# peterzjx/DeepHall

Hardware: AMD Instinct MI355X
Metric: local-energies/sec + MCMC walker-steps/sec, N=6 2Q=15, 1/2/4/8 GPUs (higher is better)
Workload: dtype f32; 1 GPU; VMC iteration (mcmc_step 10 MH moves + local energy + stats all-reduce), nspins=[6, 0] flux=15, Psiformer 4x64 heads, 2 layers, 1 det; walkers_per_gpu=4096, global_batch=4096, parallelism=walker-dp1, walker_groups_per_gpu=1, gemm_arithmetic=x6all

## Files before the change

deephall_amd/_lib.py:

```python

from __future__ import annotations

import ctypes as C
import os
from pathlib import Path

LIB_PATH = Path(__file__).resolve().parent / "_lib" / "libdeephall_amd.so"

DH_NSTATS = 16
STAT_NAMES = [
    "energy_re",
    "energy_im",
    "clipped_re",
    "clipped_im",
    "ere2",
    "kinetic_re",
    "kinetic_im",
    "potential",
    "angular_momentum_z",
    "angular_momentum_z_square",
    "angular_momentum_square",
    "pmove",
    "nvalid",
    "clipped_lz2",
# ... 18 lines not shown
    "dh_loss_diff",
    "dh_init_walkers",
    "dh_potential",
    "dh_histograms",
    "dh_monopole_orbitals",
    "dh_mh_init",
    "dh_mh_propose",
    "dh_mh_accept",
    "dh_kinetic_from_derivatives",
    "dh_debug_trunk",
    "dh_debug_gemm",
    "dh_debug_gemm_ln",
    "dh_debug_gemm_x6_ln",
    "dh_debug_chain_x6",
    "dh_debug_gemm_lnch",
    "dh_debug_set_lnch_form",
    "dh_debug_x6_plane_rows",
    "dh_debug_split_planes",
    "dh_debug_gemm_x6",
    "dh_debug_gemm_x6_choice",
    "dh_debug_route",
    "dh_debug_set_det_in_chain",
    "dh_debug_det_in_chain",
    "dh_ref_layout",
    "dh_set_params_ref",
    "dh_vjp_workspace_bytes",
    "dh_logpsi_vjp",
    "dh_grad_cotangent",
    "dh_adam_update",
    "dh_profile_enable",
    "dh_profile_read",
    "dh_debug_f_offset",
    "dh_debug_env_leaf",
    "dh_kfac_layout",
    "dh_kfac_workspace_bytes",
    "dh_kfac_vjp",
    "dh_kfac_step",
    "dh_ntk_workspace_bytes",
    "dh_ntk_tile_walkers",
    "dh_ntk",
    "dh_ntk_part",
    "dh_ntk_mirror",
    "dh_ntk_owner",
    "dh_minsr_matrix_workspace_bytes",
    "dh_minsr_matrix",
    "dh_ntk_jvp_workspace_bytes",
# ... 95 lines not shown
    lib.dh_debug_gemm_ln.restype = i32
    lib.dh_debug_gemm_x6_ln.argtypes = [i32, i32, vp, i32, vp, i32, vp, vp, vp, i32, i32, vp]
    lib.dh_debug_gemm_x6_ln.restype = i32
    lib.dh_debug_chain_x6.argtypes = [vp, vp, i32, vp, vp, vp, i32, vp, vp, vp, i32, vp, i32, vp, i32, vp, i32, vp]
    lib.dh_debug_chain_x6.restype = i32
    lib.dh_debug_gemm_lnch.argtypes = [i32, i32, vp, vp, i32, vp, vp, vp, vp, i32, vp]
    lib.dh_debug_gemm_lnch.restype = i32
    lib.dh_debug_set_lnch_form.argtypes = [i32]
    lib.dh_debug_set_lnch_form.restype = i32
    lib.dh_debug_x6_plane_rows.argtypes = [i32]
    lib.dh_debug_x6_plane_rows.restype = i32
    lib.dh_debug_split_planes.argtypes = [vp, i32, i32, i32, vp, vp]
    lib.dh_debug_split_planes.restype = i32
    lib.dh_debug_gemm_x6.argtypes = [i32, vp, i32, vp, i32, vp, vp, i32, vp, i32, i32, i32, i32, i32, vp]
    lib.dh_debug_gemm_x6.restype = i32
    lib.dh_debug_gemm_x6_choice.argtypes = [i32, i32]
    lib.dh_debug_gemm_x6_choice.restype = i32
    lib.dh_debug_route.argtypes = [vp, i32, i32, C.POINTER(i32), i32]
    lib.dh_debug_route.restype = i32
    lib.dh_debug_set_det_in_chain.argtypes = [i32]
    lib.dh_debug_set_det_in_chain.restype = i32
    lib.dh_debug_det_in_chain.argtypes = [vp, i32, i32]
    lib.dh_debug_det_in_chain.restype = i32
    lib.dh_ref_layout.argtypes = [vp, C.POINTER(sz), i32]
    lib.dh_ref_layout.restype = i32
    lib.dh_set_params_ref.argtypes = [vp, vp, sz, vp]
    lib.dh_set_params_ref.restype = i32
    lib.dh_vjp_workspace_bytes.argtypes = [vp, i32]
    lib.dh_vjp_workspace_bytes.restype = sz
    lib.dh_logpsi_vjp.argtypes = [vp, vp, i32, vp, vp, vp, vp, sz, vp]
    lib.dh_logpsi_vjp.restype = i32
    lib.dh_kfac_layout.argtypes = [vp, C.POINTER(sz), i32]
    lib.dh_kfac_layout.restype = i32
    lib.dh_kfac_workspace_bytes.argtypes = [vp, i32]
    lib.dh_kfac_workspace_bytes.restype = sz
    lib.dh_kfac_vjp.argtypes = [vp, vp, i32, vp, vp, vp, vp, vp, sz, vp]
    lib.dh_kfac_vjp.restype = i32
    lib.dh_kfac_step.argtypes = [vp, vp, vp, f32, f32, vp, vp, f32, f32, f32, vp, vp, vp, sz, vp]
    lib.dh_kfac_step.restype = i32
    lib.dh_ntk_workspace_bytes.argtypes = [vp, i32]
    lib.dh_ntk_workspace_bytes.restype = sz
    lib.dh_ntk_tile_walkers.argtypes = [vp]
    lib.dh_ntk_tile_walkers.restype = i32
    lib.dh_ntk.argtypes = [vp, vp, i32, vp, vp, vp, vp, sz, vp]
    lib.dh_ntk.restype = i32
    lib.dh_ntk_part.argtypes = [vp, vp, i32, vp, vp, vp, vp, sz, i32, i32, vp]
# ... 42 lines not shown
```

deephall_amd/csrc/api.cpp:

```cpp
#include <cmath>
#include <cstring>

#include "api_internal.h"

using namespace dh;

thread_local std::string dh::g_err;

namespace {

struct Work {
  float *h, *qkv, *o, *t, *F, *geo, *x2, *logpsi, *lp;
  int32_t* nacc;
  size_t total_bytes;
  TrunkRoute route;
};

size_t env_first_floats(const Dims& d, int nw) {
  const size_t ne = (size_t)nw * d.N, r6 = (size_t)round_up((int)(6 * ne), 256), r1 = (size_t)round_up((int)ne, 256);
  return align64(r6 * 256) + align64(r6 * d.ld_orb) + align64(r1 * env_first_k(d)) + align64(r1 * 256 * 2 * d.N);
}

Work carve(const Dims& d, int gemm_mode, int nw, int C, void* base) {
  const int rows = nw * d.N * C;
// ... 579 lines not shown
  return DH_OK;
}

size_t dh_workspace_bytes(const dh_handle* h, int batch, int op) {
  if (!h || batch < 1) return 0;
  return carve(h->d, h->gemm_mode, batch, op == 1 ? h->d.C : 1, nullptr).total_bytes;
}

}

namespace {

struct Trunk {
  dh_handle* h;
  const Dims& d;
  const Params& P;
  const Work& w;
  hipStream_t s;
  const int nw, C, rows;
  const TrunkRoute r;
  const bool keep_h;
  const ChainDet* det = nullptr;
  const bool keep_F = false;
  const int D = d.D, KO = ofeat_k(d);
  const int ch = C > 1 ? PK_CH : 0;
  const double R = rows, DD = D, f4 = 4.0;

  void gemm(const float* X, int ldx, const float* W, const float* Wt, const uint16_t* Wp, int ldw, const float* bias,
            const float* Res, int ldr, float* Y, int ldy, int ncols, int K) const {
    PROF(PK_GEMM + ch, 2.0 * R * ncols * K, f4 * (R * K + (double)K * ncols + R * ncols * (Res ? 2 : 1)));
    dense_gemm(r.family, X, ldx, W, Wt, Wp, ldw, bias, Res, ldr, Y, ldy, rows, ncols, K, C, s);
  }
  X6Feat h0_feat(int l) const { return (r.h0_epilogue && l == 0) ? X6Feat{P.W0, w.geo, d.N, d.n_up} : X6Feat{}; }

  void layer_chain(int l, bool attn) const {
    const LayerParams& lp = P.layer[l];
    const bool last = l + 1 == d.L;
    const int n3 = last ? d.orb_cols : 3 * D;
    PROF(PK_GEMM, 2.0 * R * DD * (2.0 * DD + n3), f4 * (2.0 * R * DD + R * n3 + 2.0 * DD * DD + DD * n3));
    X6Feat feat = h0_feat(l);
    if (attn) {
      feat.W0qkv = P.W0qkv;
      feat.bqkv = lp.bqkv;
      feat.Mqk = P.Mqk;
      feat.L1V = P.L1VP;
      feat.L1B = P.L1BP;
    }
    launch_chain_x6(w.o, attn ? P.UP : lp.WolP, x6_plane_rows(D), lp.bol, lp.ln1, lp.WmP, x6_plane_rows(D), lp.bm,
                    lp.ln2, last ? P.WorbP : P.layer[l + 1].WqkvP, x6_plane_rows(n3),
                    last ? P.borb : P.layer[l + 1].bqkv, n3, last ? w.F : w.qkv, last ? d.ld_orb : 3 * D, w.h, rows,
                    feat, s, !last || keep_h,
                    last ? det : nullptr, !(last && det) || keep_F);
  }
  void layer_ln_epilogue(int l) const {
    const LayerParams& lp = P.layer[l];
    const bool x6 = r.family == GEMM_X6;
    {
      PROF(PK_GEMM, 2.0 * R * DD * DD, f4 * (3.0 * R * DD + DD * DD));
      if (x6)
        launch_gemm_x6_ln(w.o, D, lp.WolP, x6_plane_rows(D), lp.bol, lp.ln1, w.h, rows, D, 0, 0, s, h0_feat(l));
      else
        launch_gemm_ln(w.o, D, lp.WolT, D, lp.bol, lp.ln1, w.h, rows, D, 0, 0, s);
    }
    PROF(PK_GEMM, 2.0 * R * DD * DD, f4 * (2.0 * R * DD + DD * DD));
    if (x6)
      launch_gemm_x6_ln(w.h, D, lp.WmP, x6_plane_rows(D), lp.bm, lp.ln2, w.h, rows, D, 1, 0, s);
    else
      launch_gemm_ln(w.h, D, lp.WmT, D, lp.bm, lp.ln2, w.h, rows, D, 1, 0, s);
  }
  void layer_lnch(int l) const {
    const LayerParams& lp = P.layer[l];
    {
      const bool of = r.ofeat && l == 0;
      const double KK = of ? KO : DD;
      PROF(PK_GEMM + PK_CH, 2.0 * R * DD * KK, f4 * (R * KK + 2.0 * R * DD + DD * KK));
// ... 22 lines not shown
    else
      gemm(w.o, D, lp.Wol, lp.WolT, lp.WolP, D, lp.bol, lf ? nullptr : w.h, D, w.t, D, D, D);
    {
      PROF(PK_LN + ch, 0.0, f4 * R * 2.0 * DD);
      launch_layernorm(d, w.t, nullptr, lp.ln1, w.geo, w.h, nw, C, 0, s, lf ? P.W0 : nullptr);
    }
    gemm(w.h, D, lp.Wm, lp.WmT, lp.WmP, D, lp.bm, nullptr, 0, w.o, D, D, D);
    PROF(PK_LN + ch, 0.0, f4 * R * 3.0 * DD);
    launch_layernorm(d, nullptr, w.o, lp.ln2, w.geo, w.h, nw, C, 1, s);
  }

  int run(const float* x, bool geo_ready) const {
    if (!(geo_ready && r.input_skip)) {
      const bool wq = r.input_qkv;
      PROF(PK_INPUT + ch, 8.0 * R * DD * (wq ? 4 : 1), f4 * R * DD * (wq ? 4 : 1));
      launch_input(d, x, P.W0, wq ? P.W0qkv : nullptr, wq ? P.layer[0].bqkv : nullptr, r.input_h ? w.h : nullptr,
                   wq ? w.qkv : nullptr, w.geo, nw, C, s);
    }
    for (int l = 0; l < d.L; ++l) {
      const LayerParams& lp = P.layer[l];
      const int form = l == 0 ? r.form0 : r.form1;
      if (l > 0 && r.qkv_gemm)
        gemm(w.h, D, lp.Wqkv, lp.WqkvT, lp.WqkvP, 3 * D, lp.bqkv, nullptr, 0, w.qkv, 3 * D, 3 * D, D);
      if (form != LF_CHAIN_ATTN) {
        const bool f = r.attn_feat && l == 0;
        PROF(PK_ATTN + ch, 0.0, f4 * R * (f ? 1.0 : 4.0) * DD);
        launch_attention(d, w.qkv, w.geo, w.o, nw, C, s, f ? P.W0qkv : nullptr, f ? lp.bqkv : nullptr,
                         f ? P.Mqk : nullptr);
      }
      switch (form) {
        case LF_CHAIN:
        case LF_CHAIN_ATTN: layer_chain(l, form == LF_CHAIN_ATTN); break;
        case LF_LN_EPILOGUE: layer_ln_epilogue(l); break;
        case LF_LNCH_WHOLE: layer_lnch_whole(); break;
        case LF_LNCH_PAIR: layer_lnch(l); break;
        case LF_L1CH: layer_l1ch(); break;
        default: layer_separate(l); break;
      }
    }
    if (r.orbital == ORB_GEMM)
      gemm(w.h, D, P.Worb, P.WorbT, P.WorbP, d.ld_orb, P.borb, nullptr, 0, w.F, d.ld_orb, d.orb_cols, D);
    return check_launch();
  }
};

int run_trunk(dh_handle* h, const float* x, int nw, int C, const Work& w, hipStream_t s, bool geo_ready = false,
              bool keep_h = false, const ChainDet* det = nullptr, bool keep_F = false) {
  return Trunk{h, h->d, h->p, w, s, nw, C, nw * h->d.N * C, w.route, keep_h, det, keep_F}.run(x, geo_ready);
}

ChainDet chain_det(const dh_handle* h, const float* x, int nw, float* logpsi, const McmcEpi& epi) {
  const Dims& d = h->d;
  ChainDet c;
  c.x = x;
  c.jastrow = h->p.jastrow;
  c.norm = h->norm;
  c.logpsi = logpsi;
  c.N = d.N;
  c.n_up = d.n_up;
  c.M = d.M;
  c.K = d.K;
  c.nw = nw;
  c.per = det_value_per(d);
  c.ldf = det_chain_ldf(d);
  c.epi = epi;
  return c;
}

int launch_trial(dh_handle* h, const float* x, float* logpsi, float* e_l, float* obs, int nw, hipStream_t s) {
  if (!h->expo && !h->expo_host.empty()) {
    HIP_TRY(hipMalloc(&h->expo, h->expo_host.size() * sizeof(int)));
    HIP_TRY(hipMemcpy(h->expo, h->expo_host.data(), h->expo_host.size() * sizeof(int), hipMemcpyHostToDevice));
  }
  PROF(e_l ? PK_DET_ENERGY : PK_DET_VALUE, 0.0, e_l ? 48.0 * nw : 8.0 * nw * h->d.N);
  if (h->state == dh_handle::PFAFFIAN)
    launch_pfaffian(h->d, x, h->cfg.cf_flux, logpsi, e_l, obs, nw, s);
  else if (h->state == dh_handle::JAIN)
    launch_cf(h->d, x, h->expo, h->cf_dense, logpsi, e_l, obs, nw, s);
  else
    launch_laughlin(h->d, x, h->expo, logpsi, e_l, obs, nw, s);
  return check_launch();
}

int value_pass(dh_handle* h, const float* x, int nw, const Work& w, float* logpsi, hipStream_t s,
               bool geo_ready = false, const McmcEpi& epi = McmcEpi{}) {
  if (h->analytic()) return launch_trial(h, x, logpsi, nullptr, nullptr, nw, s);
  if (w.route.det_in_chain && !h->prof.on) {
    const ChainDet det = chain_det(h, x, nw, logpsi, epi);
    return run_trunk(h, x, nw, 1, w, s, geo_ready, false, &det);
  }
  if (int rc = run_trunk(h, x, nw, 1, w, s, geo_ready)) return rc;
  {
    PROF(PK_DET_VALUE, 0.0, 4.0 * nw * h->d.N * h->d.ld_orb);
    launch_det_value(h->d, w.F, x, h->p.jastrow, h->norm, logpsi, nw, s, epi);
  }
  return check_launch();
}

}

extern "C" {

int dh_logpsi(dh_handle* h, const float* x, int B, float* logpsi, void* ws, size_t ws_bytes, void* stream) {
  const size_t need = h ? dh_workspace_bytes(h, B, 0) : 0;
  if (int rc = check_common(h, x, B, ws, ws_bytes, need)) return rc;
  if (!logpsi) return fail(DH_EINVAL, "null output");
  hipStream_t s = (hipStream_t)stream;
  Work w = carve(h->d, h->gemm_mode, B, 1, ws);
  return value_pass(h, x, B, w, logpsi, s);
}

int dh_mcmc_step(dh_handle* h, float* x, float* lp, int32_t* n_accept, int B, int steps, float width, uint64_t seed,
                 uint64_t counter, int64_t walker_offset, const float* noise, void* ws, size_t ws_bytes,
                 void* stream) {
// ... 124 lines not shown

int dh_fidelity_partial(const float* logpsi, const float* logphi, int B, double* part, void* stream) {
  if (!logpsi || !logphi || !part) return fail(DH_EINVAL, "dh_fidelity_partial: null argument");
  if (B < 1) return fail(DH_EINVAL, "dh_fidelity_partial needs B >= 1");
  launch_fidelity_partial(logpsi, logphi, B, part, (hipStream_t)stream);
  return check_launch();
}

int dh_fidelity_residual(const float* logpsi, const float* logphi, int B, const double* total, float* resid,
                         void* stream) {
  if (!logpsi || !logphi || !total || !resid) return fail(DH_EINVAL, "dh_fidelity_residual: null argument");
  if (B < 1) return fail(DH_EINVAL, "dh_fidelity_residual needs B >= 1");
  launch_fidelity_residual(logpsi, logphi, B, total, resid, (hipStream_t)stream);
  return check_launch();
}

int dh_debug_trunk(dh_handle* h, const float* x, int B, int op, void* ws, size_t ws_bytes, void* stream) {
  const size_t need = h ? dh_workspace_bytes(h, B, op) : 0;
  if (int rc = check_common(h, x, B, ws, ws_bytes, need)) return rc;
  Work w = carve(h->d, h->gemm_mode, B, op == 1 ? h->d.C : 1, ws);
  if (!w.F)
    return fail(DH_EINVAL, "dh_debug_trunk: this config's local energy goes envelope first and maps no orbital "
                           "features F over the channel rows");
  if (op != 1 && w.route.det_in_chain) {
    const ChainDet det = chain_det(h, x, B, w.logpsi, McmcEpi{});
    return run_trunk(h, x, B, 1, w, (hipStream_t)stream, false, true, &det, true);
  }
  return run_trunk(h, x, B, op == 1 ? h->d.C : 1, w, (hipStream_t)stream, false, true);
}

int dh_debug_env_leaf(const float* thph, int n, int M, int sq, float* out, void* stream) {
  if (!thph || !out || n < 1 || M < 1) return fail(DH_EINVAL, "bad env_leaf probe args");
  launch_env_leaf_probe(thph, n, M, sq, out, (hipStream_t)stream);
  return check_launch();
}

size_t dh_debug_f_offset(const dh_handle* h, int B, int op) {
  if (!h || B < 1) return (size_t)-1;
  Work w = carve(h->d, h->gemm_mode, B, op == 1 ? h->d.C : 1, reinterpret_cast<void*>(size_t(64)));
  if (!w.F) return (size_t)-1;
  return (size_t)(w.F - reinterpret_cast<float*>(size_t(64)));
}

int dh_debug_gemm(int variant, const float* X, int ldx, const float* W, int ldw, const float* bias, const float* R,
                  int ldr, float* Y, int ldy, int rows, int ncols, int K, int C, void* stream) {
  bool known = true;
  if (variant >= 100) {
    if (K % 32 != 0) return fail(DH_EINVAL, "NT GEMM needs K % 32 == 0");
    known = launch_gemm_nt_variant(variant - 100, X, ldx, W, ldw, bias, R, ldr, Y, ldy, rows, ncols, K, C,
                                   (hipStream_t)stream);
  } else {
// ... 49 lines not shown
    return fail(DH_EINVAL, "bad chain_x6 args");
  launch_chain_x6(X1, Wp1, ldp1, b1, ln1, Wp2, ldp2, b2, ln2, Wp3, ldp3, b3, n3, Y3, ldy3, h, rows, X6Feat{},
                  (hipStream_t)stream);
  return check_launch();
}

int dh_debug_gemm_lnch(int N, int mode, const float* X, const uint16_t* Wp, int ldp, const float* bias,
                       const float* ln, const float* geo, float* h, int ne, void* stream) {
  if (!gemm_lnch_supported(N, 256) || (mode != 0 && mode != 1) || (mode == 0 && !X) || !Wp || !ln || !geo || !h ||
      ne < 1 || ldp < x6_plane_rows(256) || ne % N)
    return fail(DH_EINVAL, "bad gemm_lnch args");
  launch_gemm_lnch(N, mode == 0 ? X : h, Wp, ldp, bias, ln, geo, h, ne, mode, (hipStream_t)stream);
  return check_launch();
}

int dh_debug_set_lnch_form(int form) { return set_lnch_form(form); }

int dh_debug_set_det_in_chain(int on) { return set_det_in_chain(on); }

int dh_debug_det_in_chain(const dh_handle* h, int B, int op) {
  if (!h || h->analytic() || B < 1) return fail(DH_EINVAL, "bad route query");
  const int C = op == 1 ? h->d.C : 1;
  return trunk_route(h->d, h->gemm_mode, C, B * h->d.N * C).det_in_chain;
}

int dh_debug_gemm_ln(int mode, int bm, const float* X, int ldx, const float* Wt, int ldw, const float* bias,
                     const float* ln, float* h, int rows, int K, void* stream) {
  if (!gemm_ln_supported(256, K) || rows < 1 || (mode != 0 && mode != 1)) return fail(DH_EINVAL, "bad gemm_ln args");
  launch_gemm_ln(X, ldx, Wt, ldw, bias, ln, h, rows, K, mode, bm, (hipStream_t)stream);
  return check_launch();
}

int dh_profile_enable(dh_handle* h, int on) {
  if (!h) return fail(DH_EINVAL, "null handle");
  h->prof.on = on != 0;
  h->prof.used = 0;
  return DH_OK;
}

int dh_profile_read(dh_handle* h, double* out, int reset) {
  if (!h || !out) return fail(DH_EINVAL, "null argument");
  for (int i = 0; i < 4 * PK_TOTAL; ++i) out[i] = 0.0;
  for (size_t i = 0; i < h->prof.used; ++i) {
    ProfRec& r = h->prof.recs[i];
    HIP_TRY(hipEventSynchronize(r.b));
    float ms = 0.f;
// ... 73 lines not shown
```

deephall_amd/csrc/attn_val.h:

```cpp
#pragma once
#include "device_common.h"

namespace dh {

struct FeatW {
  float4 wq, wk, wv;
  float bq, bk, bv;
  __device__ void load(const float* W0qkv, const float* bqkv, int D, int col) {
    const int ld = 3 * D;
    wq = make_float4(W0qkv[col], W0qkv[ld + col], W0qkv[2 * ld + col], W0qkv[3 * ld + col]);
    wk = make_float4(W0qkv[D + col], W0qkv[ld + D + col], W0qkv[2 * ld + D + col], W0qkv[3 * ld + D + col]);
    wv = make_float4(W0qkv[2 * D + col], W0qkv[ld + 2 * D + col], W0qkv[2 * ld + 2 * D + col],
                     W0qkv[3 * ld + 2 * D + col]);
    bq = bqkv[col];
    bk = bqkv[D + col];
    bv = bqkv[2 * D + col];
  }
  __device__ __forceinline__ static float dot(float4 f, float4 w) {
    return fmaf(f.x, w.x, fmaf(f.y, w.y, fmaf(f.z, w.z, f.w * w.w)));
  }
};

template <int N>
__device__ __forceinline__ void feat_qkv(const FeatW& fw, const float* __restrict__ geo, int b, int n_up,
                                         float (&pq)[N], float (&pk)[N], float (&pv)[N]) {
#pragma unroll
  for (int i = 0; i < N; ++i) {
    const float4 g = *reinterpret_cast<const float4*>(geo + 4 * (size_t)(b * N + i));
    const float4 f = make_float4(g.y, g.x * g.w, g.x * g.z, (i < n_up) ? 1.f : -1.f);
    pq[i] = FeatW::dot(f, fw.wq) + fw.bq;
    pk[i] = FeatW::dot(f, fw.wk) + fw.bk;
    pv[i] = FeatW::dot(f, fw.wv) + fw.bv;
  }
}

template <int N>
__host__ __device__ constexpr int attn_val_floats() { return 2 * N * 68 + N * N; }

template <int N, int NT>
__device__ __forceinline__ void attn_val_core(const float (&pq)[NT][N], const float (&pk)[NT][N],
                                              const float (&pv)[NT][N], float* st, int lane, float (&out)[NT][N]) {
  constexpr int ld = 68, nn = N * N, PER = attn_val_floats<N>();
  __builtin_amdgcn_wave_barrier();
#pragma unroll
  for (int t = 0; t < NT; ++t)
#pragma unroll
    for (int i = 0; i < N; ++i) {
      st[t * PER + i * ld + lane] = pq[t][i];
      st[t * PER + N * ld + i * ld + lane] = pk[t][i];
    }
  __builtin_amdgcn_wave_barrier();
  for (int p = lane; p < NT * 4 * nn; p += 64) {
    const int t = p / (4 * nn), pp = p - t * (4 * nn);
    const int pair = pp >> 2, qt = pp & 3, i = pair / N, j = pair - (pair / N) * N;
    const float* x = st + t * PER + i * ld + 16 * qt;
    const float* y = st + t * PER + N * ld + j * ld + 16 * qt;
    float sdot = 0.f;
#pragma unroll
    for (int m = 0; m < 4; ++m) {
      const float4 a = *reinterpret_cast<const float4*>(x + 4 * m);
      const float4 c = *reinterpret_cast<const float4*>(y + 4 * m);
      sdot = fmaf(a.x, c.x, fmaf(a.y, c.y, fmaf(a.z, c.z, fmaf(a.w, c.w, sdot))));
    }
    sdot += __shfl_xor(sdot, 1, 64);
    sdot += __shfl_xor(sdot, 2, 64);
    if (qt == 0) st[t * PER + 2 * N * ld + pair] = sdot * 0.125f;
  }
  __builtin_amdgcn_wave_barrier();
  if (lane < NT * N) {
    const int t = lane / N, r = lane - t * N;
    float* A = st + t * PER + 2 * N * ld + r * N;
    float m = -INFINITY;
#pragma unroll
    for (int j = 0; j < N; ++j) m = fmaxf(m, A[j]);
// ... 153 lines not shown
```

deephall_amd/csrc/dh_internal.h:

```cpp
#pragma once
#include <algorithm>
#include <hip/hip_runtime.h>
#include <stdint.h>
#include <stddef.h>

#include "../../include/deephall_amd.h"

namespace dh {

struct Dims {
  int N, n_up, n_dn;
  int T;
  int C;
  int M;
  float Q, r;
  int H, dh, D, L, K;
  int NB;
  int orb_cols;
  int ld_orb;
  int interaction;
  float lambda;
  int sparse;
};
constexpr int kSparseFeatures = 8;
// ... 37 lines not shown
  LF_SEPARATE = 0,
  LF_LN_EPILOGUE,
  LF_CHAIN,
  LF_CHAIN_ATTN,
  LF_LNCH_PAIR,
  LF_LNCH_WHOLE,
  LF_L1CH,
};
enum OrbitalMap : int { ORB_NONE = 0, ORB_GEMM = 1, ORB_IN_CHAIN = 2 };
enum DetStage : int { DET_VALUE = 0, DET_DIRECT = 1, DET_PRECONTRACT = 2, DET_ENV_FIRST = 3 };
struct TrunkRoute {
  int family;
  int input_h;
  int input_qkv;
  int input_skip;
  int form0, form1;
  int attn_feat;
  int h0_epilogue;
  int ofeat;
  int qkv_gemm;
  int orbital;
  int det;
  int det_in_chain;
};
constexpr int kTrunkRouteFields = 12;
static_assert(sizeof(TrunkRoute) == (kTrunkRouteFields + 1) * sizeof(int) &&
                  offsetof(TrunkRoute, det_in_chain) == kTrunkRouteFields * sizeof(int),
              "dh_debug_route copies the first kTrunkRouteFields fields as ints");
int gemm_family(const Dims& d, bool want_x6);
TrunkRoute trunk_route(const Dims& d, int gemm_mode, int C, int rows);
int set_det_in_chain(int on);

constexpr int kChainTileRows = 96;
constexpr size_t kChainPlaneBytes = 3 * (size_t)kChainTileRows * 264 * 2;
inline int det_value_per(const Dims& d) {
  return (2 * d.N * d.M + 2 * d.N * d.N + 2 * d.N + 2 * d.K + 2 + 4 + 6 * d.N + 2 + 3 + 1) & ~3;
}
inline bool det_value_half_wave(const Dims& d) {
  const int mgv = (d.M + 64 / d.N - 1) / (64 / d.N);
  return mgv <= 2 && d.N * d.N <= 64;
}
inline int det_chain_ldf(const Dims& d) {
  return d.orb_cols + (((d.N * d.K - d.orb_cols) % 32) + 32) % 32;
}

constexpr int kRowPad = 256;
constexpr int kWalkerRowPad = 768;
inline int round_up(int a, int b) { return (a + b - 1) / b * b; }

template <typename Kern>
inline void ensure_smem(Kern kernel, size_t bytes) {
  if (bytes > 65536)
    (void)hipFuncSetAttribute(reinterpret_cast<const void*>(kernel), hipFuncAttributeMaxDynamicSharedMemorySize,
                              (int)bytes);
// ... 31 lines not shown
void launch_gemm_x6(const float* X, int ldx, const uint16_t* Wp, int ldp, const float* bias, const float* R, int ldr,
                    float* Y, int ldy, int rows, int ncols, int K, int C, hipStream_t s);
struct X6Feat {
  const float* W0 = nullptr;
  const float* geo = nullptr;
  int N = 1, n_up = 0;
  const float* W0qkv = nullptr;
  const float* bqkv = nullptr;
  const float* Mqk = nullptr;
  const uint16_t* L1V = nullptr;
  const uint16_t* L1B = nullptr;
};
bool launch_gemm_x6_ln(const float* X, int ldx, const uint16_t* Wp, int ldp, const float* bias, const float* ln,
                       float* h, int rows, int K, int mode, int nw, hipStream_t s, X6Feat feat = X6Feat{});
bool gemm_lnch_supported(int N, int D);
int set_lnch_form(int f);
void launch_gemm_lnch(int N, const float* X, const uint16_t* Wp, int ldp, const float* bias, const float* ln,
                      const float* geo, float* h, int ne, int mode, hipStream_t s,
                      const float* W0f = nullptr, int n_up = 0, int K = 256, const uint16_t* Wv = nullptr,
                      const uint16_t* Wb = nullptr);
void launch_l1_basis(const Dims& d, const float* W0, const float* UT, const float* bol, const float* ln1,
                     const float* Wm, const float* bm, float* BT, float* VT, hipStream_t s);
bool chain_attn_supported(int N, int H, int dh);
struct ChainDet;
void launch_chain_x6(const float* X1, const uint16_t* Wp1, int ldp1, const float* b1, const float* ln1,
                     const uint16_t* Wp2, int ldp2, const float* b2, const float* ln2, const uint16_t* Wp3, int ldp3,
                     const float* b3, int n3, float* Y3, int ldy3, float* h, int rows, X6Feat feat, hipStream_t s,
                     bool store_h = true, const ChainDet* det = nullptr, bool store_F = true);
void launch_transpose(const float* src, int ld_src, int rows, int cols, float* dst, int ld_dst, hipStream_t s);

void launch_input(const Dims& d, const float* x, const float* W0, const float* W0qkv, const float* bqkv, float* h,
                  float* qkv, float* geo, int nw, int C, hipStream_t s);
void launch_propose(const Dims& d, const float* x, float* x2, int nw, float width, uint64_t seed, uint64_t step,
                    int64_t walker_offset, const float* noise, int noise_stride, hipStream_t s, float* geo = nullptr);
void launch_accept_propose(const Dims& d, float* x, float* x2, float* geo, float* lp, const float* logpsi2,
                           int32_t* n_acc, int nw, float width, uint64_t seed, uint64_t step, int64_t walker_offset,
                           const float* noise, const float* noise2, hipStream_t s);
void launch_init_walkers(const Dims& d, float* x, int nw, uint64_t seed, int64_t walker_offset, hipStream_t s);

bool attention_takes_features(const Dims& d, int C);
bool attention_mfma_supported(const Dims& d);
void launch_attention_mfma(const Dims& d, const float* qkv, const float* geo, float* o, int nw, hipStream_t s,
                           const float* W0qkv, const float* bqkv);
void launch_attention(const Dims& d, const float* qkv, const float* geo, float* o, int nw, int C, hipStream_t s,
                      const float* W0qkv = nullptr, const float* bqkv = nullptr, const float* Mqk = nullptr);
void launch_lowrank_qk(const Dims& d, const float* W0qkv, const float* bqkv, float* Mqk, hipStream_t s);
void launch_ofeat_weight(const Dims& d, const float* W0qkv, const float* bqkv, const float* Wol, float* UT,
                         hipStream_t s);

void launch_layernorm(const Dims& d, const float* X, const float* Z, const float* ln, const float* geo, float* h,
                      int nw, int C, int mode, hipStream_t s,
// ... 188 lines not shown
```

deephall_amd/csrc/gemm_x6.hip:

```cpp
#include <cstdlib>
#include <type_traits>

#include "attn_val.h"
#include "dh_internal.h"
#include "device_common.h"
#include "det_value.h"

#ifndef CHAIN_STAMP
#define CHAIN_STAMP 0
#endif

namespace dh {

#if CHAIN_STAMP
constexpr int CHAIN_STAMP_WG = 512, CHAIN_NSTAMP = 16;
__device__ unsigned long long g_chain_stamp[2 * CHAIN_STAMP_WG * CHAIN_NSTAMP];
#define CHAIN_T(i)                                                                                  \
  do {                                                                                              \
    if (threadIdx.x == 0 && blockIdx.x < CHAIN_STAMP_WG)                                            \
      g_chain_stamp[((NA > 0) * CHAIN_STAMP_WG + blockIdx.x) * CHAIN_NSTAMP + (i)] = __builtin_amdgcn_s_memtime(); \
  } while (0)
extern "C" int dh_debug_chain_stamps(unsigned long long* out, int n) {
  n = n < 2 * CHAIN_STAMP_WG * CHAIN_NSTAMP ? n : 2 * CHAIN_STAMP_WG * CHAIN_NSTAMP;
  return hipMemcpyFromSymbol(out, HIP_SYMBOL(g_chain_stamp), n * sizeof(unsigned long long)) == hipSuccess ? 0 : -1;
// ... 1007 lines not shown
constexpr int CS_PRMF = 5 * 256;
constexpr size_t CS_PLANE = (size_t)CH_BM * CS_LSP * 2, CS_SMEM = 3 * CS_PLANE + 2 * CS_NW * CH_BM * 4 + CS_PRMF * 4;
static_assert(CS_SMEM <= 163840, "chain LDS");
static_assert(CH_BM == kChainTileRows && 3 * CS_PLANE == kChainPlaneBytes, "trunk_route's LDS bound of the determinant tail");

__device__ __forceinline__ void split4(const float4& x, uint2& h, uint2& m, uint2& l) {
  const float a[4] = {x.x, x.y, x.z, x.w};
  uint32_t H[2], Mv[2], Lv[2];
#pragma unroll
  for (int p = 0; p < 2; ++p) {
    const float u = a[2 * p], v = a[2 * p + 1];
    const uint32_t h2 = pk_bf16(u, v);
    const float ru = u - lo_f(h2), rv = v - hi_f(h2);
    const uint32_t m2 = pk_bf16(ru, rv);
    H[p] = h2;
    Mv[p] = m2;
    Lv[p] = pk_bf16(ru - lo_f(m2), rv - hi_f(m2));
  }
  h = make_uint2(H[0], H[1]);
  m = make_uint2(Mv[0], Mv[1]);
  l = make_uint2(Lv[0], Lv[1]);
}

constexpr int kChainDet = -1;
template <int NAT = 0>
__global__ __launch_bounds__(512) void chain_x6s_kernel(ChainArgs a) {
  constexpr bool DET = NAT == kChainDet;
  constexpr int NA = DET ? 0 : NAT;
  constexpr int RB = CS_RB, PD = CS_PD, LSP = CS_LSP;
  using K16 = std::integral_constant<int, CH_K / 16>;
  using KP1 = std::integral_constant<int, (NA > 0 ? CH_KO / 16 : CH_K / 16)>;
  using K2 = std::integral_constant<int, 2>;
  extern __shared__ float4 smem4[];
  char* smem = reinterpret_cast<char*>(smem4);
  float* part = reinterpret_cast<float*>(smem + 3 * CS_PLANE);
  float* prm = part + 2 * CS_NW * CH_BM;
  const int tid = threadIdx.x, lane = tid & 63;
  const int wid = __builtin_amdgcn_readfirstlane(tid >> 6);
  const int l32 = lane & 31, lh = lane >> 5;
  int bid = blockIdx.x;
  {
    const int nblk = gridDim.x, q = nblk / 8, r8 = nblk % 8, xcd = bid % 8, slot = bid / 8;
    bid = (xcd < r8 ? xcd * (q + 1) : r8 * (q + 1) + (xcd - r8) * q) + slot;
  }
  constexpr int TRW = NA > 0 ? (CH_BM / NA) * NA : CH_BM;
  const int row0 = bid * TRW, rows = min(a.rows, row0 + TRW);
  auto lbar = []() __attribute__((always_inline)) {
    asm volatile("s_waitcnt lgkmcnt(0)" ::: "memory");
    __builtin_amdgcn_s_barrier();
    asm volatile("" ::: "memory");
  };
// ... 205 lines not shown
#pragma unroll
      for (int q = 0; q < 5; ++q) {
        float acc1 = 0.f;
#pragma unroll
        for (int j = 0; j < NA; ++j) acc1 = fmaf(A[j], *stg(F_ + 5 * (w * NA + j) + q), acc1);
        ov[q] = live ? acc1 : 0.f;
      }
    }
    lbar();
    if (act) {
      const int r = w * NA + i;
#pragma unroll
      for (int q = 0; q < 8; ++q) {
        const float x = q < 5 ? ov[q] : 0.f;
        const uint32_t h2 = pk_bf16(x, 0.f);
        const float rx = x - lo_f(h2);
        const uint32_t m2 = pk_bf16(rx, 0.f);
        const uint32_t l2 = pk_bf16(rx - lo_f(m2), 0.f);
        const int c = 8 * hh + q;
        *reinterpret_cast<uint16_t*>(pl(0, r, c)) = (uint16_t)h2;
        *reinterpret_cast<uint16_t*>(pl(1, r, c)) = (uint16_t)m2;
        *reinterpret_cast<uint16_t*>(pl(2, r, c)) = (uint16_t)l2;
      }
    }
    lbar();
  } else {
    prefetch(a.Wp1, a.ldp1, 0, KP1{});
    const float4* src = reinterpret_cast<const float4*>(a.X1 + (size_t)row0 * CH_K);
#pragma unroll 4
    for (int i = tid; i < CH_BM * (CH_K / 4); i += 512) {
      const int r = i / (CH_K / 4), c = 4 * (i % (CH_K / 4));
      put4(r, c, src[i]);
    }
    lbar();
  }
  CHAIN_T(1);
  gemm(NoTr{}, KP1{}, Zero{});
  CHAIN_T(2);
  {
    float4 bvv[4];
#pragma unroll
    for (int g = 0; g < 4; ++g) bvv[g] = *reinterpret_cast<const float4*>(a.b1 + colof(g));
    if (a.feat.W0) {
      float4 w0[4][4];
#pragma unroll
      for (int g = 0; g < 4; ++g)
// ... 387 lines not shown
  }
#define DH_X6LN(TNV, NWV, WNV)                                                                               \
  do {                                                                                                       \
    if (mode == 0)                                                                                           \
      launch_x6d_t<TNV, NWV, 3, 1, WNV>(X, ldx, Wp, ldp, bias, h, 256, h, 256, rows, 256, K, 1, s, ln, feat); \
    else                                                                                                     \
      launch_x6d_t<TNV, NWV, 3, 2, WNV>(X, ldx, Wp, ldp, bias, h, 256, h, 256, rows, 256, K, 1, s, ln);      \
  } while (0)
  switch (nw) {
    case 1: DH_X6LN(2, 3, 4); break;
    case 2: DH_X6LN(2, 2, 4); break;
    case 3: DH_X6LN(8, 3, 1); break;
    case 4: DH_X6LN(8, 4, 1); break;
    case 8: DH_X6LN(2, 4, 4); break;
    default: return false;
  }
#undef DH_X6LN
  return true;
}

void launch_chain_x6(const float* X1, const uint16_t* Wp1, int ldp1, const float* b1, const float* ln1,
                     const uint16_t* Wp2, int ldp2, const float* b2, const float* ln2, const uint16_t* Wp3, int ldp3,
                     const float* b3, int n3, float* Y3, int ldy3, float* h, int rows, X6Feat feat, hipStream_t s,
                     bool store_h, const ChainDet* det, bool store_F) {
  ChainArgs a{X1, Wp1, Wp2, Wp3, ldp1, ldp2, ldp3, b1, ln1, b2, ln2, b3, n3, ldy3, Y3, h, rows, feat, store_h ? 1 : 0,
              store_F ? 1 : 0, det ? *det : ChainDet{}};
  auto k = chain_x6s_kernel<0>;
  if (det) k = chain_x6s_kernel<kChainDet>;
  if (feat.W0qkv) {
    switch (feat.N) {
      case 2: k = chain_x6s_kernel<2>; break;
      case 3: k = chain_x6s_kernel<3>; break;
      case 4: k = chain_x6s_kernel<4>; break;
      case 6: k = chain_x6s_kernel<6>; break;
      case 8: k = chain_x6s_kernel<8>; break;
      case 10: k = chain_x6s_kernel<10>; break;
      default: k = chain_x6s_kernel<20>; break;
    }
  }
  const int trw = feat.W0qkv ? (CH_BM / feat.N) * feat.N : CH_BM;
  ensure_smem(k, CS_SMEM);
  hipLaunchKernelGGL(k, dim3((rows + trw - 1) / trw), dim3(512), CS_SMEM, s, a);
}

bool chain_attn_supported(int N, int H, int dh) {
  return H == 4 && dh == 64 && (N == 2 || N == 3 || N == 4 || N == 6 || N == 8 || N == 10 || N == 20);
}

}
```

deephall_amd/csrc/trunk_route.cpp:

```cpp
#include <atomic>

#include "dh_internal.h"

namespace dh {

namespace {
std::atomic<int> g_det_in_chain{1};
}
int set_det_in_chain(int on) { return g_det_in_chain.exchange(on ? 1 : 0); }

int gemm_family(const Dims& d, bool want_x6) {
  const bool nt = d.D % 32 == 0;
  return nt && want_x6 && gemm_x6_supported(d.D) ? GEMM_X6 : nt ? GEMM_F32_NT : GEMM_F32_NN;
}

TrunkRoute trunk_route(const Dims& d, int gemm_mode, int C, int rows) {
  const int D = d.D;
  const bool channels = C > 1;
  const bool unfused = gemm_mode == DH_GEMM_X6_ALL_UNFUSED;
  TrunkRoute r{};
  r.family = gemm_family(d, channels ? gemm_mode != DH_GEMM_F32 : (gemm_mode == DH_GEMM_X6_ALL || unfused));
  const bool x6 = r.family == GEMM_X6, nt = r.family != GEMM_F32_NN;
  const bool fused = d.L > 0 && attention_takes_features(d, C);
  r.attn_feat = fused;
  r.input_qkv = d.L > 0 && !fused;
  r.qkv_gemm = 1;
  r.form0 = r.form1 = LF_SEPARATE;
  r.det = !channels ? DET_VALUE : env_first(d) ? DET_ENV_FIRST : det_precontract(d) ? DET_PRECONTRACT : DET_DIRECT;
  r.orbital = r.det == DET_ENV_FIRST ? ORB_NONE : ORB_GEMM;

  if (!channels && nt && gemm_ln_supported(D, D)) {
    r.form0 = r.form1 = LF_LN_EPILOGUE;
// ... 2 lines not shown
      r.form0 = fused && chain_attn_supported(d.N, d.H, d.dh) ? LF_CHAIN_ATTN : LF_CHAIN;
      r.form1 = LF_CHAIN;
      r.ofeat = r.form0 == LF_CHAIN_ATTN;
      r.qkv_gemm = 0;
      r.orbital = ORB_IN_CHAIN;
    }
  } else if (channels) {
    r.ofeat = fused;
    if (x6 && C == 2 * d.N + 5 && !unfused && gemm_lnch_supported(d.N, D)) {
      r.form0 = fused && d.H == 4 ? LF_LNCH_WHOLE : LF_LNCH_PAIR;
      r.form1 = LF_LNCH_PAIR;
      r.h0_epilogue = fused;
    } else if (fused && D == 256 && (d.N == 10 || d.N == 20)) {
      r.h0_epilogue = 1;
      if (d.dh == 64 && d.H == 4 && layer1_ch_supported(d) && !unfused) r.form0 = LF_L1CH;
    }
  }
  r.input_h = !r.h0_epilogue;
  r.input_skip = !channels && r.h0_epilogue;
  const int last_form = d.L > 1 ? r.form1 : r.form0;
  r.det_in_chain = g_det_in_chain.load() && !channels && d.L > 0 && last_form == LF_CHAIN && r.orbital == ORB_IN_CHAIN &&
                   det_value_half_wave(d) && kChainTileRows % d.N == 0 && d.orb_cols <= 256 &&
                   (size_t)kChainTileRows * det_chain_ldf(d) * 4 + 16 * (size_t)det_value_per(d) * 4 <= kChainPlaneBytes;
  return r;
}

}
```

include/deephall_amd.h:

```cpp
#ifndef DEEPHALL_AMD_H
#define DEEPHALL_AMD_H

#include <stddef.h>
#include <stdint.h>

#ifdef __cplusplus
extern "C" {
#endif

#define DH_OK 0
#define DH_EINVAL -1
#define DH_EHIP -2
#define DH_ENOMEM -3
#define DH_ESTATE -4

#define DH_INTERACTION_COULOMB 0
#define DH_INTERACTION_HARMONIC 1
#define DH_NETWORK_PSIFORMER 0
#define DH_NETWORK_LAUGHLIN 1
#define DH_NETWORK_JAIN 2
#define DH_NETWORK_PFAFFIAN 3
#define DH_ORBITAL_FULL 0
#define DH_ORBITAL_SPARSE 1

// ... 128 lines not shown

int dh_debug_trunk(dh_handle* h, const float* x, int B, int op, void* ws, size_t ws_bytes, void* stream);
size_t dh_debug_f_offset(const dh_handle* h, int B, int op);
int dh_debug_env_leaf(const float* thph, int n, int M, int sq, float* out, void* stream);
int dh_debug_gemm(int variant, const float* X, int ldx, const float* W, int ldw, const float* bias, const float* R,
                  int ldr, float* Y, int ldy, int rows, int ncols, int K, int C, void* stream);

int dh_debug_gemm_ln(int mode, int bm, const float* X, int ldx, const float* Wt, int ldw, const float* bias,
                     const float* ln, float* h, int rows, int K, void* stream);

int dh_debug_gemm_x6_ln(int mode, int nw, const float* X, int ldx, const uint16_t* Wp, int ldp, const float* bias,
                        const float* ln, float* h, int rows, int K, void* stream);
int dh_debug_chain_x6(const float* X1, const uint16_t* Wp1, int ldp1, const float* b1, const float* ln1,
                      const uint16_t* Wp2, int ldp2, const float* b2, const float* ln2, const uint16_t* Wp3,
                      int ldp3, const float* b3, int n3, float* Y3, int ldy3, float* h, int rows, void* stream);

int dh_debug_gemm_lnch(int N, int mode, const float* X, const uint16_t* Wp, int ldp, const float* bias,
                       const float* ln, const float* geo, float* h, int ne, void* stream);

int dh_debug_gemm_x6_choice(int rows, int ncols);
int dh_debug_route(const dh_handle* h, int B, int op, int* out, int n);
int dh_debug_set_det_in_chain(int on);
int dh_debug_det_in_chain(const dh_handle* h, int B, int op);
int dh_debug_x6_plane_rows(int ncols);
int dh_debug_split_planes(const float* Wt, int ldw, int ncols, int K, uint16_t* Wp, void* stream);
int dh_debug_gemm_x6(int variant, const float* X, int ldx, const uint16_t* Wp, int ldp, const float* bias,
                     const float* R, int ldr, float* Y, int ldy, int rows, int ncols, int K, int C, void* stream);

int dh_init_walkers(dh_handle* h, float* x, int B, uint64_t seed, int64_t walker_offset, void* stream);

#ifdef __cplusplus
}
#endif
#endif
```

Baseline: 832,900 local-energies/s.

## Fuse later-layer attention into the x6 chain kernel prologue

For layers after the first, the attention-value step is computed inside the chain GEMM kernel. The kernel reads q/k/v straight from the qkv buffer and writes the result as split bf16 planes into shared memory, so the separate attention launch and the o-buffer round trip through global memory go away. An ILP variant of the score loop with float4 loads and DPP reductions is added for this path. The change costs extra kernel template instantiations, more register and shared-memory pressure, and an aliasing assert between the qkv input and the output. The path is on by default and can be turned off through a debug toggle.

```diff
diff --git a/deephall_amd/_lib.py b/deephall_amd/_lib.py
--- a/deephall_amd/_lib.py
+++ b/deephall_amd/_lib.py
@@ -64,6 +64,8 @@
     "dh_debug_route",
     "dh_debug_set_det_in_chain",
     "dh_debug_det_in_chain",
+    "dh_debug_set_attn_in_chain",
+    "dh_debug_attn_in_chain",
     "dh_ref_layout",
     "dh_set_params_ref",
     "dh_vjp_workspace_bytes",
@@ -205,6 +207,10 @@
     lib.dh_debug_set_det_in_chain.restype = i32
     lib.dh_debug_det_in_chain.argtypes = [vp, i32, i32]
     lib.dh_debug_det_in_chain.restype = i32
+    lib.dh_debug_set_attn_in_chain.argtypes = [i32]
+    lib.dh_debug_set_attn_in_chain.restype = i32
+    lib.dh_debug_attn_in_chain.argtypes = [vp, i32, i32]
+    lib.dh_debug_attn_in_chain.restype = i32
     lib.dh_ref_layout.argtypes = [vp, C.POINTER(sz), i32]
     lib.dh_ref_layout.restype = i32
     lib.dh_set_params_ref.argtypes = [vp, vp, sz, vp]
diff --git a/deephall_amd/csrc/api.cpp b/deephall_amd/csrc/api.cpp
--- a/deephall_amd/csrc/api.cpp
+++ b/deephall_amd/csrc/api.cpp
@@ -625,6 +625,9 @@
   const bool keep_h;
   const ChainDet* det = nullptr;
   const bool keep_F = false;
+  const bool attn2 = false;
+  bool stores_F(int l) const { return !(l + 1 == d.L && det) || keep_F; }
+  bool attn2_at(int l) const { return attn2 && l > 0 && !(l + 1 == d.L && stores_F(l)); }
   const int D = d.D, KO = ofeat_k(d);
   const int ch = C > 1 ? PK_CH : 0;
   const double R = rows, DD = D, f4 = 4.0;
@@ -649,11 +652,12 @@
       feat.L1V = P.L1VP;
       feat.L1B = P.L1BP;
     }
-    launch_chain_x6(w.o, attn ? P.UP : lp.WolP, x6_plane_rows(D), lp.bol, lp.ln1, lp.WmP, x6_plane_rows(D), lp.bm,
+    const bool a2 = attn2_at(l);
+    launch_chain_x6(a2 ? w.qkv : w.o, attn ? P.UP : lp.WolP, x6_plane_rows(D), lp.bol, lp.ln1, lp.WmP, x6_plane_rows(D), lp.bm,
                     lp.ln2, last ? P.WorbP : P.layer[l + 1].WqkvP, x6_plane_rows(n3),
                     last ? P.borb : P.layer[l + 1].bqkv, n3, last ? w.F : w.qkv, last ? d.ld_orb : 3 * D, w.h, rows,
                     feat, s, !last || keep_h,
-                    last ? det : nullptr, !(last && det) || keep_F);
+                    last ? det : nullptr, stores_F(l), a2 ? d.N : 0);
   }
   void layer_ln_epilogue(int l) const {
     const LayerParams& lp = P.layer[l];
@@ -722,7 +726,7 @@
       const int form = l == 0 ? r.form0 : r.form1;
       if (l > 0 && r.qkv_gemm)
         gemm(w.h, D, lp.Wqkv, lp.WqkvT, lp.WqkvP, 3 * D, lp.bqkv, nullptr, 0, w.qkv, 3 * D, 3 * D, D);
-      if (form != LF_CHAIN_ATTN) {
+      if (form != LF_CHAIN_ATTN && !attn2_at(l)) {
         const bool f = r.attn_feat && l == 0;
         PROF(PK_ATTN + ch, 0.0, f4 * R * (f ? 1.0 : 4.0) * DD);
         launch_attention(d, w.qkv, w.geo, w.o, nw, C, s, f ? P.W0qkv : nullptr, f ? lp.bqkv : nullptr,
@@ -745,8 +749,8 @@
 };
 
 int run_trunk(dh_handle* h, const float* x, int nw, int C, const Work& w, hipStream_t s, bool geo_ready = false,
-              bool keep_h = false, const ChainDet* det = nullptr, bool keep_F = false) {
-  return Trunk{h, h->d, h->p, w, s, nw, C, nw * h->d.N * C, w.route, keep_h, det, keep_F}.run(x, geo_ready);
+              bool keep_h = false, const ChainDet* det = nullptr, bool keep_F = false, bool attn2 = false) {
+  return Trunk{h, h->d, h->p, w, s, nw, C, nw * h->d.N * C, w.route, keep_h, det, keep_F, attn2}.run(x, geo_ready);
 }
 
 ChainDet chain_det(const dh_handle* h, const float* x, int nw, float* logpsi, const McmcEpi& epi) {
@@ -785,11 +789,12 @@
 int value_pass(dh_handle* h, const float* x, int nw, const Work& w, float* logpsi, hipStream_t s,
                bool geo_ready = false, const McmcEpi& epi = McmcEpi{}) {
   if (h->analytic()) return launch_trial(h, x, logpsi, nullptr, nullptr, nw, s);
+  const bool attn2 = w.route.attn_in_chain && !h->prof.on;
   if (w.route.det_in_chain && !h->prof.on) {
     const ChainDet det = chain_det(h, x, nw, logpsi, epi);
-    return run_trunk(h, x, nw, 1, w, s, geo_ready, false, &det);
-  }
-  if (int rc = run_trunk(h, x, nw, 1, w, s, geo_ready)) return rc;
+    return run_trunk(h, x, nw, 1, w, s, geo_ready, false, &det, false, attn2);
+  }
+  if (int rc = run_trunk(h, x, nw, 1, w, s, geo_ready, false, nullptr, false, attn2)) return rc;
   {
     PROF(PK_DET_VALUE, 0.0, 4.0 * nw * h->d.N * h->d.ld_orb);
     launch_det_value(h->d, w.F, x, h->p.jastrow, h->norm, logpsi, nw, s, epi);
@@ -960,11 +965,12 @@
   if (!w.F)
     return fail(DH_EINVAL, "dh_debug_trunk: this config's local energy goes envelope first and maps no orbital "
                            "features F over the channel rows");
+  const bool attn2 = op != 1 && w.route.attn_in_chain && !h->prof.on;
   if (op != 1 && w.route.det_in_chain) {
     const ChainDet det = chain_det(h, x, B, w.logpsi, McmcEpi{});
-    return run_trunk(h, x, B, 1, w, (hipStream_t)stream, false, true, &det, true);
-  }
-  return run_trunk(h, x, B, op == 1 ? h->d.C : 1, w, (hipStream_t)stream, false, true);
+    return run_trunk(h, x, B, 1, w, (hipStream_t)stream, false, true, &det, true, attn2);
+  }
+  return run_trunk(h, x, B, op == 1 ? h->d.C : 1, w, (hipStream_t)stream, false, true, nullptr, false, attn2);
 }
 
 int dh_debug_env_leaf(const float* thph, int n, int M, int sq, float* out, void* stream) {
@@ -1060,6 +1066,14 @@
   if (!h || h->analytic() || B < 1) return fail(DH_EINVAL, "bad route query");
   const int C = op == 1 ? h->d.C : 1;
   return trunk_route(h->d, h->gemm_mode, C, B * h->d.N * C).det_in_chain;
+}
+
+int dh_debug_set_attn_in_chain(int on) { return set_attn_in_chain(on); }
+
+int dh_debug_attn_in_chain(const dh_handle* h, int B, int op) {
+  if (!h || h->analytic() || B < 1) return fail(DH_EINVAL, "bad route query");
+  const int C = op == 1 ? h->d.C : 1;
+  return trunk_route(h->d, h->gemm_mode, C, B * h->d.N * C).attn_in_chain;
 }
 
 int dh_debug_gemm_ln(int mode, int bm, const float* X, int ldx, const float* Wt, int ldw, const float* bias,
diff --git a/deephall_amd/csrc/attn_val.h b/deephall_amd/csrc/attn_val.h
--- a/deephall_amd/csrc/attn_val.h
+++ b/deephall_amd/csrc/attn_val.h
@@ -37,7 +37,7 @@
 template <int N>
 __host__ __device__ constexpr int attn_val_floats() { return 2 * N * 68 + N * N; }
 
-template <int N, int NT>
+template <int N, int NT, bool ILP = false>
 __device__ __forceinline__ void attn_val_core(const float (&pq)[NT][N], const float (&pk)[NT][N],
                                               const float (&pv)[NT][N], float* st, int lane, float (&out)[NT][N]) {
   constexpr int ld = 68, nn = N * N, PER = attn_val_floats<N>();
@@ -50,6 +50,27 @@
       st[t * PER + N * ld + i * ld + lane] = pk[t][i];
     }
   __builtin_amdgcn_wave_barrier();
+  if constexpr (ILP) {
+    constexpr int TOT = NT * 4 * nn;
+#pragma unroll
+    for (int it = 0; it < (TOT + 63) / 64; ++it) {
+      const int p0 = lane + 64 * it, p = p0 < TOT ? p0 : TOT - 1;
+      const int t = p / (4 * nn), pp = p - t * (4 * nn);
+      const int pair = pp >> 2, qt = pp & 3, i = pair / N, j = pair - (pair / N) * N;
+      const float* x = st + t * PER + i * ld + 16 * qt;
+      const float* y = st + t * PER + N * ld + j * ld + 16 * qt;
+      float sdot = 0.f;
+#pragma unroll
+      for (int m = 0; m < 4; ++m) {
+        const float4 a = *reinterpret_cast<const float4*>(x + 4 * m);
+        const float4 c = *reinterpret_cast<const float4*>(y + 4 * m);
+        sdot = fmaf(a.x, c.x, fmaf(a.y, c.y, fmaf(a.z, c.z, fmaf(a.w, c.w, sdot))));
+      }
+      sdot += dpp_mov<0xB1>(sdot);
+      sdot += dpp_mov<0x4E>(sdot);
+      if (qt == 0 && p0 < TOT) st[t * PER + 2 * N * ld + pair] = sdot * 0.125f;
+    }
+  } else
   for (int p = lane; p < NT * 4 * nn; p += 64) {
     const int t = p / (4 * nn), pp = p - t * (4 * nn);
     const int pair = pp >> 2, qt = pp & 3, i = pair / N, j = pair - (pair / N) * N;
diff --git a/deephall_amd/csrc/dh_internal.h b/deephall_amd/csrc/dh_internal.h
--- a/deephall_amd/csrc/dh_internal.h
+++ b/deephall_amd/csrc/dh_internal.h
@@ -83,14 +83,16 @@
   int orbital;
   int det;
   int det_in_chain;
+  int attn_in_chain;
 };
 constexpr int kTrunkRouteFields = 12;
-static_assert(sizeof(TrunkRoute) == (kTrunkRouteFields + 1) * sizeof(int) &&
+static_assert(sizeof(TrunkRoute) == (kTrunkRouteFields + 2) * sizeof(int) &&
                   offsetof(TrunkRoute, det_in_chain) == kTrunkRouteFields * sizeof(int),
               "dh_debug_route copies the first kTrunkRouteFields fields as ints");
 int gemm_family(const Dims& d, bool want_x6);
 TrunkRoute trunk_route(const Dims& d, int gemm_mode, int C, int rows);
 int set_det_in_chain(int on);
+int set_attn_in_chain(int on);
 
 constexpr int kChainTileRows = 96;
 constexpr size_t kChainPlaneBytes = 3 * (size_t)kChainTileRows * 264 * 2;
@@ -168,11 +170,12 @@
 void launch_l1_basis(const Dims& d, const float* W0, const float* UT, const float* bol, const float* ln1,
                      const float* Wm, const float* bm, float* BT, float* VT, hipStream_t s);
 bool chain_attn_supported(int N, int H, int dh);
+bool chain_attn2_supported(int N, int H, int dh);
 struct ChainDet;
 void launch_chain_x6(const float* X1, const uint16_t* Wp1, int ldp1, const float* b1, const float* ln1,
                      const uint16_t* Wp2, int ldp2, const float* b2, const float* ln2, const uint16_t* Wp3, int ldp3,
                      const float* b3, int n3, float* Y3, int ldy3, float* h, int rows, X6Feat feat, hipStream_t s,
-                     bool store_h = true, const ChainDet* det = nullptr, bool store_F = true);
+                     bool store_h = true, const ChainDet* det = nullptr, bool store_F = true, int attn2_n = 0);
 void launch_transpose(const float* src, int ld_src, int rows, int cols, float* dst, int ld_dst, hipStream_t s);
 
 void launch_input(const Dims& d, const float* x, const float* W0, const float* W0qkv, const float* bqkv, float* h,
diff --git a/deephall_amd/csrc/gemm_x6.hip b/deephall_amd/csrc/gemm_x6.hip
--- a/deephall_amd/csrc/gemm_x6.hip
+++ b/deephall_amd/csrc/gemm_x6.hip
@@ -1,3 +1,4 @@
+#include <cassert>
 #include <cstdlib>
 #include <type_traits>
 
@@ -1053,11 +1054,12 @@
   l = make_uint2(Lv[0], Lv[1]);
 }
 
-constexpr int kChainDet = -1;
+constexpr int kChainDet = -1, kChainAttn2 = 100;
 template <int NAT = 0>
 __global__ __launch_bounds__(512) void chain_x6s_kernel(ChainArgs a) {
-  constexpr bool DET = NAT == kChainDet;
-  constexpr int NA = DET ? 0 : NAT;
+  constexpr int N2 = NAT >= kChainAttn2 ? NAT - kChainAttn2 : (NAT <= -kChainAttn2 ? -NAT - kChainAttn2 : 0);
+  constexpr bool DET = NAT == kChainDet || NAT <= -kChainAttn2;
+  constexpr int NA = (DET || N2 > 0) ? 0 : NAT;
   constexpr int RB = CS_RB, PD = CS_PD, LSP = CS_LSP;
   using K16 = std::integral_constant<int, CH_K / 16>;
   using KP1 = std::integral_constant<int, (NA > 0 ? CH_KO / 16 : CH_K / 16)>;
@@ -1309,6 +1311,78 @@
         *reinterpret_cast<uint16_t*>(pl(1, r, c)) = (uint16_t)m2;
         *reinterpret_cast<uint16_t*>(pl(2, r, c)) = (uint16_t)l2;
       }
+    }
+    lbar();
+  } else if constexpr (N2 > 0) {
+    constexpr int NT = 2;
+    constexpr int WT = CH_BM / N2, WH = WT / 2, NR = WH / NT;
+    constexpr int PER = attn_val_floats<N2>(), WST = (NT * PER + 3) & ~3;
+    static_assert(CS_NW == 8 && CH_BM % N2 == 0 && WT % 4 == 0 && WH * N2 == 48, "4 heads x 2 walker halves of whole pairs");
+    constexpr size_t ST_BYTES = (size_t)CS_NW * WST * 4;
+    constexpr bool EARLY = ST_BYTES <= CS_PLANE + 2 * CS_NW * CH_BM * 4;
+    static_assert(ST_BYTES <= 3 * CS_PLANE, "staging fits the planes");
+    prefetch(a.Wp1, a.ldp1, 0, KP1{});
+    const int hh = wid & 3, wl0 = WH * (wid >> 2);
+    float* st = reinterpret_cast<float*>(smem + (EARLY ? 2 * CS_PLANE : 0)) + wid * WST;
+    const float* qb = a.X1 + (size_t)(row0 + wl0 * N2) * (3 * CH_K) + 64 * hh + lane;
+    auto ldq = [&](int rd, float(&q)[NT][N2], float(&k)[NT][N2], float(&v)[NT][N2]) __attribute__((always_inline)) {
+#pragma unroll
+      for (int t = 0; t < NT; ++t)
+#pragma unroll
+        for (int i = 0; i < N2; ++i) {
+          const float* p = qb + (size_t)((NT * rd + t) * N2 + i) * (3 * CH_K);
+          q[t][i] = p[0];
+          k[t][i] = p[CH_K];
+          v[t][i] = p[2 * CH_K];
+        }
+    };
+    const bool odd = lane & 1;
+    const int cp = 64 * hh + (lane & ~1);
+    uint32_t H[WH * N2 / 2], M[WH * N2 / 2], L[WH * N2 / 2];
+    float pq[2][NT][N2], pk[2][NT][N2], pv[2][NT][N2];
+    ldq(0, pq[0], pk[0], pv[0]);
+#pragma unroll
+    for (int rd = 0; rd < NR; ++rd) {
+      if (rd + 1 < NR) ldq(rd + 1, pq[(rd + 1) & 1], pk[(rd + 1) & 1], pv[(rd + 1) & 1]);
+      __builtin_amdgcn_sched_barrier(0);
+      float out[NT * N2] = {};
+      if (row0 + (wl0 + NT * rd) * N2 < rows) {
+        float o2[NT][N2];
+        attn_val_core<N2, NT, true>(pq[rd & 1], pk[rd & 1], pv[rd & 1], st, lane, o2);
+#pragma unroll
+        for (int t = 0; t < NT; ++t) {
+          const bool live = row0 + (wl0 + NT * rd + t) * N2 < rows;
+#pragma unroll
+          for (int i = 0; i < N2; ++i) out[t * N2 + i] = live ? o2[t][i] : 0.f;
+        }
+      }
+#pragma unroll
+      for (int e = 0; e < NT * N2; e += 2) {
+        const float got = dpp_mov<0xB1>(odd ? out[e] : out[e + 1]);
+        const float u = odd ? got : out[e], v = odd ? out[e + 1] : got;
+        const uint32_t h2 = pk_bf16(u, v);
+        const float ru = u - lo_f(h2), rv = v - hi_f(h2);
+        const uint32_t m2 = pk_bf16(ru, rv);
+        const int q = (NT * N2 * rd + e) / 2;
+        H[q] = h2;
+        M[q] = m2;
+        L[q] = pk_bf16(ru - lo_f(m2), rv - hi_f(m2));
+        if constexpr (EARLY) {
+          const int r = wl0 * N2 + 2 * q + odd;
+          *reinterpret_cast<uint32_t*>(pl(0, r, cp)) = h2;
+          *reinterpret_cast<uint32_t*>(pl(1, r, cp)) = m2;
+        }
+      }
+    }
+    lbar();
+#pragma unroll
+    for (int q = 0; q < WH * N2 / 2; ++q) {
+      const int r = wl0 * N2 + 2 * q + odd;
+      if constexpr (!EARLY) {
+        *reinterpret_cast<uint32_t*>(pl(0, r, cp)) = H[q];
+        *reinterpret_cast<uint32_t*>(pl(1, r, cp)) = M[q];
+      }
+      *reinterpret_cast<uint32_t*>(pl(2, r, cp)) = L[q];
     }
     lbar();
   } else {
@@ -1742,11 +1816,28 @@
 void launch_chain_x6(const float* X1, const uint16_t* Wp1, int ldp1, const float* b1, const float* ln1,
                      const uint16_t* Wp2, int ldp2, const float* b2, const float* ln2, const uint16_t* Wp3, int ldp3,
                      const float* b3, int n3, float* Y3, int ldy3, float* h, int rows, X6Feat feat, hipStream_t s,
-                     bool store_h, const ChainDet* det, bool store_F) {
+                     bool store_h, const ChainDet* det, bool store_F, int attn2_n) {
   ChainArgs a{X1, Wp1, Wp2, Wp3, ldp1, ldp2, ldp3, b1, ln1, b2, ln2, b3, n3, ldy3, Y3, h, rows, feat, store_h ? 1 : 0,
               store_F ? 1 : 0, det ? *det : ChainDet{}};
   auto k = chain_x6s_kernel<0>;
   if (det) k = chain_x6s_kernel<kChainDet>;
+  if (attn2_n) {
+    const bool stores_y3 = Wp3 && (!det || store_F);
+    const size_t xbytes = (size_t)((rows + CH_BM - 1) / CH_BM * CH_BM) * 3 * CH_K * 4, ybytes = (size_t)rows * ldy3 * 4;
+    const char *xb = reinterpret_cast<const char*>(X1), *yb = reinterpret_cast<const char*>(Y3);
+    assert(!stores_y3 || (yb == xb && ldy3 == 3 * CH_K) || yb + ybytes <= xb || xb + xbytes <= yb);
+    (void)stores_y3, (void)xbytes, (void)ybytes, (void)xb, (void)yb;
+    switch (attn2_n) {
+#define DH_ATTN2(NV) \
+  case NV: k = det ? chain_x6s_kernel<-(kChainAttn2 + NV)> : chain_x6s_kernel<kChainAttn2 + NV>; break
+      DH_ATTN2(2);
+      DH_ATTN2(3);
+      DH_ATTN2(4);
+      DH_ATTN2(6);
+      default: DH_ATTN2(8);
+#undef DH_ATTN2
+    }
+  }
   if (feat.W0qkv) {
     switch (feat.N) {
       case 2: k = chain_x6s_kernel<2>; break;
@@ -1767,4 +1858,8 @@
   return H == 4 && dh == 64 && (N == 2 || N == 3 || N == 4 || N == 6 || N == 8 || N == 10 || N == 20);
 }
 
-}
+bool chain_attn2_supported(int N, int H, int dh) {
+  return H == 4 && dh == 64 && (N == 2 || N == 3 || N == 4 || N == 6 || N == 8);
+}
+
+}
diff --git a/deephall_amd/csrc/trunk_route.cpp b/deephall_amd/csrc/trunk_route.cpp
--- a/deephall_amd/csrc/trunk_route.cpp
+++ b/deephall_amd/csrc/trunk_route.cpp
@@ -5,9 +5,10 @@
 namespace dh {
 
 namespace {
-std::atomic<int> g_det_in_chain{1};
+std::atomic<int> g_det_in_chain{1}, g_attn_in_chain{1};
 }
 int set_det_in_chain(int on) { return g_det_in_chain.exchange(on ? 1 : 0); }
+int set_attn_in_chain(int on) { return g_attn_in_chain.exchange(on ? 1 : 0); }
 
 int gemm_family(const Dims& d, bool want_x6) {
   const bool nt = d.D % 32 == 0;
@@ -56,6 +57,8 @@
   r.det_in_chain = g_det_in_chain.load() && !channels && d.L > 0 && last_form == LF_CHAIN && r.orbital == ORB_IN_CHAIN &&
                    det_value_half_wave(d) && kChainTileRows % d.N == 0 && d.orb_cols <= 256 &&
                    (size_t)kChainTileRows * det_chain_ldf(d) * 4 + 16 * (size_t)det_value_per(d) * 4 <= kChainPlaneBytes;
+  r.attn_in_chain = g_attn_in_chain.load() && !channels && r.form1 == LF_CHAIN && d.L > 1 && kChainTileRows % d.N == 0 &&
+                    chain_attn2_supported(d.N, d.H, d.dh);
   return r;
 }
 
diff --git a/include/deephall_amd.h b/include/deephall_amd.h
--- a/include/deephall_amd.h
+++ b/include/deephall_amd.h
@@ -174,6 +174,8 @@
 int dh_debug_route(const dh_handle* h, int B, int op, int* out, int n);
 int dh_debug_set_det_in_chain(int on);
 int dh_debug_det_in_chain(const dh_handle* h, int B, int op);
+int dh_debug_set_attn_in_chain(int on);
+int dh_debug_attn_in_chain(const dh_handle* h, int B, int op);
 int dh_debug_x6_plane_rows(int ncols);
 int dh_debug_split_planes(const float* Wt, int ldw, int ncols, int K, uint16_t* Wp, void* stream);
 int dh_debug_gemm_x6(int variant, const float* X, int ldx, const uint16_t* Wp, int ldp, const float* bias,
```

Result: no change. 833,700 local-energies/s, median of 2 (+0.1%).
